# yewsiang/Transferable3D

Measured on AMD Instinct MI355X. Metric: frustums/sec fwd+bwd, higher is better.
Workload: dtype f32

## Files before the change

include/t3d.h:

```cpp
#ifndef T3D_H_
#define T3D_H_

#include <stdint.h>

#ifdef __cplusplus
extern "C" {
#endif

#define T3D_OK 0
#define T3D_ERR_ARG (-1)
#define T3D_ERR_SHAPE (-2)
#define T3D_ERR_LAUNCH (-3)
#define T3D_ERR_ABI (-4)

#define T3D_ABI_VERSION 3
#define T3D_V2_SIZE_pointmlp_fwd_args 200
#define T3D_V2_SIZE_pointmlp_dgrad_args 168
#define T3D_V2_SIZE_pointmlp_wgrad_args 144
#define T3D_V2_SIZE_pointmlp_dgrad_gram_args 168
#define T3D_V2_SIZE_pointmlp_gram_args 96
#define T3D_V2_SIZE_seg_head_args 208
#define T3D_V2_SIZE_boxpc_rep_args 104

#define T3D_TILE_ROWS 128
// ... 694 lines not shown
  float bn_init_decay, bn_decay_rate, bn_decay_step, bn_decay_clip;
  float beta1, beta2;
  int batch_size;
  int step_offset;
} t3d_schedule;
int t3d_schedule_step(float* hyper, const t3d_schedule* s, t3d_stream_t stream);

int t3d_adam_tf_step(float* params, const float* grads, float* m, float* v, int64_t n,
                     const float* hyper, float beta1, float beta2, float eps, float grad_scale,
                     t3d_stream_t stream);

typedef struct { int64_t off; int64_t n; int32_t blk0; int32_t reserved; } t3d_adam_range;
int t3d_reduce_slabs_adam(const float* slab_base, float* grad_base, const t3d_slab_desc* table_dev, int n_tensors, int max_numel,
                          float* params, float* m, float* v, const t3d_adam_range* ranges_dev, int n_ranges, int n_range_blocks,
                          const float* hyper, float beta1, float beta2, float eps, float grad_scale, t3d_stream_t stream);

int t3d_split_x3(const float* src, void* planes, int64_t n, int64_t plane_stride, t3d_stream_t stream);

typedef struct {
  int64_t off;
  int32_t K, N;
  int32_t fwd, dgrad;
  int32_t blk0;
  int32_t reserved;
} t3d_x3_frag_entry;
int t3d_split_x3_frag(const float* params, void* planes_fwd, void* planes_dgrad, int64_t plane_stride, const t3d_x3_frag_entry* table,
                      int n_entries, int n_blocks, t3d_stream_t stream);

int t3d_step_head_takes(const t3d_pointmlp_fwd_args* fwd);
int t3d_step_head(const t3d_pointmlp_fwd_args* fwd, const float* params, void* planes_fwd, void* planes_dgrad, int64_t plane_stride,
                  const t3d_x3_frag_entry* table, int n_entries, int n_blocks, float* hyper, const t3d_schedule* sched,
                  t3d_stream_t stream);

int t3d_momentum_step(float* params, const float* grads, float* accum, int64_t n, const float* hyper, float momentum,
                      float grad_scale, t3d_stream_t stream);

typedef struct {
  t3d_act_src a;
  const float* mask;
  float keep_prob;
  float* out;
  int M, K;
  int rows_per_frustum;
} t3d_act_dropout_args;
int t3d_act_dropout(const t3d_act_dropout_args* args, t3d_stream_t stream);

int t3d_cast_bf16(const float* src, void* dst, int64_t n, t3d_stream_t stream);

int t3d_dropout_mask(float* mask, int64_t n, float keep_prob, uint32_t seed, const float* hyper,
                     t3d_stream_t stream);

enum { T3D_SMALL_BN_BWD_FINALIZE = 1, T3D_SMALL_FC_BWD = 2, T3D_SMALL_FC_DINPUT = 3, T3D_SMALL_DY_COLSUM = 4,
       T3D_SMALL_BN_FWD_FINALIZE = 5, T3D_SMALL_FC_FWD = 6, T3D_SMALL_POOL_BWD_MID = 7 };
typedef struct {
  const float* slab_base;
  float* grad_base;
  const t3d_slab_desc* table_dev;
  int n_tensors, max_numel;
  t3d_pool_sparse_rows_args sparse;
} t3d_pool_bwd_mid_args;
typedef struct {
  int kind;
  int depends;
  union {
    t3d_bn_bwd_finalize_args bn_bwd;
    t3d_fc_bwd_args fc_bwd;
// ... 350 lines not shown
```

transferable3d_amd/abi.py:

```python
import ctypes as C
import os

F = C.POINTER(C.c_float)
I = C.POINTER(C.c_int32)
D = C.POINTER(C.c_double)
L = C.POINTER(C.c_int64)
i32, f32 = C.c_int, C.c_float

TILE_ROWS = 128
F32, BF16 = 0, 1
DTYPE_BY_NAME = {'f32': F32, 'bf16': BF16}
ARITH_AUTO, ARITH_FP32_MFMA, ARITH_BF16X3, ARITH_BF16 = 0, 1, 2, 3
ARITH_BY_NAME = {'auto': ARITH_AUTO, 'fp32_mfma': ARITH_FP32_MFMA, 'bf16x3': ARITH_BF16X3}
ARITH_NAMES = {ARITH_FP32_MFMA: 'fp32_mfma', ARITH_BF16X3: 'bf16x3', ARITH_BF16: 'bf16'}
ABI_VERSION = 3
ERR_ABI = -4
ACT_NONE, ACT_RELU, ACT_LEAKY_RELU, ACT_TANH = 0, 1, 2, 3
ACT_BY_NAME = {None: ACT_NONE, 'relu': ACT_RELU, 'leaky_relu': ACT_LEAKY_RELU, 'tanh': ACT_TANH}


class Sized(C.Structure):

    def __init__(self, *args, **kw):
        super().__init__(C.sizeof(type(self)), *args, **kw)
# ... 7 lines not shown
class DySrc(C.Structure):
    _fields_ = [('dz', F), ('y', F), ('coef', F), ('argidx', I), ('dpool', F), ('dtype', i32)]


class PointMlpFwdArgs(Sized):
    _fields_ = [('struct_size', C.c_uint32), ('a', ActSrc), ('w', F), ('bias', F), ('rowbias', F), ('y', F), ('psum', F), ('psumsq', F),
                ('rowmask', F), ('pmax', F), ('pmin', F), ('pamax', I), ('pamin', I),
                ('M', i32), ('K', i32), ('N', i32), ('rows_per_frustum', i32), ('dtype', i32), ('w_x3', C.c_void_p), ('w_x3_stride', C.c_int64), ('arith', i32)]


class BnFwdFinalizeArgs(C.Structure):
    _fields_ = [('psum', F), ('psumsq', F), ('n_tiles', i32), ('count', i32), ('N', i32), ('gamma', F), ('beta', F),
                ('moving_mean', F), ('moving_var', F), ('decay', F), ('eps', f32), ('is_training', i32),
                ('unbiased_ema', i32), ('scale', F), ('shift', F), ('mean', F), ('invstd', F),
                ('pool_pmax', F), ('pool_pmin', F), ('pool_pamax', I), ('pool_pamin', I), ('pool_B', i32), ('pool_tiles_per_frustum', i32),
                ('pooled', F), ('ld_pooled', i32), ('argidx', I), ('ysel', F)]


class PoolFinalizeArgs(C.Structure):
    _fields_ = [('scale', F), ('shift', F), ('pmax', F), ('pmin', F), ('pamax', I), ('pamin', I),
                ('B', i32), ('N', i32), ('tiles_per_frustum', i32), ('pooled', F), ('ld_pooled', i32),
                ('argidx', I), ('ysel', F)]


class PointMlpDgradArgs(Sized):
    _fields_ = [('struct_size', C.c_uint32), ('dy', DySrc), ('w', F), ('add_in', F), ('prev_y', F), ('prev_scale', F), ('prev_shift', F),
                ('out', F), ('psum_dz', F), ('psum_dzy', F), ('M', i32), ('K', i32), ('N', i32),
                ('rows_per_frustum', i32), ('dtype', i32), ('w_x3', C.c_void_p), ('w_x3_stride', C.c_int64), ('arith', i32)]


class PointMlpWgradArgs(Sized):
    _fields_ = [('struct_size', C.c_uint32), ('a', ActSrc), ('dy', DySrc), ('slabs', F), ('M', i32), ('K', i32), ('N', i32),
                ('rows_per_frustum', i32), ('rows_per_split', i32), ('arith', i32)]


class PoolBwdPrepArgs(C.Structure):
    _fields_ = [('w', F), ('bias', F), ('coef', F), ('K', i32), ('N', i32), ('p_slabs', F), ('rc_slabs', F), ('wc', F)]


class PoolSparseRowsArgs(C.Structure):
    _fields_ = [('argidx', I), ('dpool', F), ('wc', F), ('B', i32), ('N', i32), ('K', i32), ('rows_per_frustum', i32), ('s', F),
                ('row_live', I)]


class PointMlpDgradGramArgs(Sized):
    _fields_ = [('struct_size', C.c_uint32), ('a', ActSrc), ('p', F), ('rowconst', F), ('add_in', F), ('add_live', I), ('prev_y', F), ('prev_scale', F),
                ('prev_shift', F),
                ('out', F), ('psum_dz', F), ('psum_dzy', F), ('M', i32), ('K', i32), ('rows_per_frustum', i32), ('dtype', i32), ('arith', i32)]


class PointMlpGramArgs(Sized):
    _fields_ = [('struct_size', C.c_uint32), ('a', ActSrc), ('slabs', F), ('M', i32), ('K', i32), ('rows_per_frustum', i32), ('rows_per_split', i32), ('arith', i32)]


class ActColsumArgs(C.Structure):
    _fields_ = [('a', ActSrc), ('M', i32), ('K', i32), ('rows_per_frustum', i32), ('part', F)]


class PoolWgradFinishArgs(C.Structure):
    _fields_ = [('a', ActSrc), ('argidx', I), ('dpool', F), ('coef', F), ('w', F), ('bias', F), ('g', F), ('abar', F),
                ('B', i32), ('K', i32), ('N', i32), ('rows_per_frustum', i32), ('dw', F)]


class BoxRefineStepArgs(C.Structure):
    _fields_ = [('out9', F), ('center_in', F), ('dims_in', F), ('theta_in', F), ('center_out', F), ('dims_out', F), ('theta_out', F),
                ('total', F), ('fit_prob', F), ('weigh_by_conf', i32), ('first', i32), ('B', i32)]
# ... 445 lines not shown
    't3d_act_colsum': [C.POINTER(ActColsumArgs), VP],
    't3d_pool_wgrad_finish': [C.POINTER(PoolWgradFinishArgs), VP],
    't3d_batch_assemble': [C.POINTER(BatchAssembleArgs), VP],
    't3d_box_refine_step': [C.POINTER(BoxRefineStepArgs), VP],
    't3d_box_refine_step_bwd': [C.POINTER(BoxRefineStepBwdArgs), VP],
    't3d_boxpc_perturb': [C.POINTER(BoxPcPerturbArgs), VP],
    't3d_sample_equal_classes': [C.POINTER(SampleEqualClassesArgs), VP],
    't3d_box3d_iou': [C.POINTER(Box3dIouArgs), VP],
    't3d_box3d_iou_corners': [C.POINTER(Box3dIouCornersArgs), VP],
    't3d_box_head_iou': [C.POINTER(BoxHeadIouArgs), VP],
    't3d_box2d_feats': [C.POINTER(Box2dFeatsArgs), VP],
    't3d_pool_bwd_stage1': [C.POINTER(PointMlpGramArgs), C.POINTER(ActColsumArgs), C.POINTER(PoolBwdPrepArgs), VP],
    't3d_pool_bwd_mid': [F, F, C.POINTER(SlabDesc), i32, i32, C.POINTER(PoolSparseRowsArgs), VP],
    't3d_pool_bwd_stage2': [C.POINTER(PoolWgradFinishArgs), C.POINTER(PointMlpDgradGramArgs), VP],
    't3d_fc_fwd': [C.POINTER(FcFwdArgs), VP],
    't3d_fc_bwd': [C.POINTER(FcBwdArgs), VP],
    't3d_fc_dinput': [C.POINTER(FcDinputArgs), VP],
    't3d_seg_head': [C.POINTER(SegHeadArgs), VP],
    't3d_seg_finalize': [C.POINTER(SegFinalizeArgs), VP],
    't3d_act_dropout': [C.POINTER(ActDropoutArgs), VP],
    't3d_strong_loss': [C.POINTER(StrongLossArgs), VP],
    't3d_boxpc_rep': [C.POINTER(BoxPcRepArgs), VP],
    't3d_boxpc_rep_b': [C.POINTER(BoxPcRepBArgs), VP],
    't3d_boxpc_rep_bwd': [C.POINTER(BoxPcRepBwdArgs), VP],
    't3d_boxpc_loss': [C.POINTER(BoxPcLossArgs), VP],
    't3d_pointmlp_dgrad_narrow': [C.POINTER(DgradNarrowArgs), VP],
    't3d_semi_final_loss': [C.POINTER(SemiFinalLossArgs), VP],
    't3d_anchor_reg_bwd': [C.POINTER(AnchorRegBwdArgs), VP],
    't3d_reduce_slabs': [F, F, C.POINTER(SlabDesc), i32, i32, VP],
    't3d_schedule_step': [F, C.POINTER(Schedule), VP],
    't3d_reduce_slabs_adam': [F, F, C.POINTER(SlabDesc), i32, i32, F, F, F, C.POINTER(AdamRange), i32, i32, F, f32, f32, f32, f32, VP],
    't3d_step_head_takes': [C.POINTER(PointMlpFwdArgs)],
    't3d_step_head': [C.POINTER(PointMlpFwdArgs), F, VP, VP, C.c_int64, VP, i32, i32, F, C.POINTER(Schedule), VP],
    't3d_adam_tf_step': [F, F, F, F, C.c_int64, F, f32, f32, f32, f32, VP],
    't3d_momentum_step': [F, F, F, C.c_int64, F, f32, f32, VP],
    't3d_split_x3': [F, VP, C.c_int64, C.c_int64, VP],
    't3d_split_x3_frag': [F, VP, VP, C.c_int64, VP, i32, i32, VP],
    't3d_dropout_mask': [F, C.c_int64, f32, C.c_uint32, F, VP],
    't3d_cast_bf16': [F, VP, C.c_int64, VP],
    't3d_frustum_extract': [C.POINTER(FrustumExtractArgs), VP],
    't3d_sunrgbd_eval': [C.POINTER(SunrgbdEvalArgs), VP],
    't3d_sunrgbd_diagnose': [C.POINTER(SunrgbdEvalArgs), C.POINTER(SunrgbdDiagnoseArgs), VP],
    't3d_detect_decode': [C.POINTER(DetectDecodeArgs), VP],
    't3d_detect_nms': [C.POINTER(DetectNmsArgs), VP],
    't3d_render': [C.POINTER(RenderArgs), VP],
    't3d_detect_consistency': [C.POINTER(DetectConsistencyArgs), VP],
    't3d_detect_fuse': [C.POINTER(DetectFuseArgs), VP],
    't3d_detect_ensemble': [C.POINTER(DetectEnsembleArgs), VP],
    't3d_detect_nms_sweep': [C.POINTER(DetectNmsSweepArgs), VP],
    't3d_sunrgbd_eval_sweep': [C.POINTER(SunrgbdEvalArgs), C.POINTER(SunrgbdSweepArgs), VP],
    't3d_semi_sample': [C.POINTER(SemiSampleArgs), VP],
    't3d_label_subset': [C.POINTER(LabelSubsetArgs), VP],
}

LIB_PATH = os.path.join(os.path.dirname(os.path.abspath(__file__)), 'libt3d.so')
ERRORS = {-1: 'T3D_ERR_ARG', -2: 'T3D_ERR_SHAPE', -3: 'T3D_ERR_LAUNCH'}


class T3DError(RuntimeError):
    pass


def source_hash_of(lib):
    buf = C.create_string_buffer(64)
    check(lib.t3d_source_hash(buf, 64), 't3d_source_hash')
    return buf.value.decode()
# ... 46 lines not shown
```

transferable3d_amd/csrc/pointmlp.hip:

```cpp
#include "common.h"
#include "poolbwd_dev.h"
#include "rider_dev.h"

#include <cstdlib>
#include <mutex>
#include <type_traits>
#include <utility>
#include <unordered_map>

namespace {

constexpr int BK = 32;
constexpr int MIN_WAVES_PER_EU = 2;
constexpr int LDR = BK + 4;
constexpr int NT = 256;

__device__ __forceinline__ float4 f4zero() { return make_float4(0.f, 0.f, 0.f, 0.f); }

__device__ __forceinline__ unsigned keep_bits32(const float* __restrict__ rowmask, int base) {
  float4 m[8];
#pragma unroll
  for (int q = 0; q < 8; ++q) m[q] = *reinterpret_cast<const float4*>(rowmask + base + (q >> 2) * 32 + (q & 3) * 8);
  unsigned bits = 0u;
#pragma unroll
// ... 2193 lines not shown
    for (int tn = 0; tn < TN; ++tn) {
      unsigned boff = ((unsigned)(k0 + wm * (BMK / 2) + 4 * h) * (unsigned)N + (unsigned)(n0 + wn * (BN / 2) + tn * 32 + l31)) * 4u;
      asm volatile("" : "+v"(boff));
#pragma unroll
      for (int tm = 0; tm < TM; ++tm)
#pragma unroll
        for (int r = 0; r < 16; ++r)
          *reinterpret_cast<float*>(sbase + (boff + (unsigned)(tm * 32 + (r & 3) + 8 * (r >> 2)) * n4)) = acc[tm][tn][r];
    }
    return;
  }
#pragma unroll
  for (int tn = 0; tn < TN; ++tn) {
    const int col = n0 + wn * (BN / 2) + tn * 32 + l31;
#pragma unroll
    for (int tm = 0; tm < TM; ++tm) {
#pragma unroll
      for (int r = 0; r < 16; ++r) {
        const int k = k0 + wm * (BMK / 2) + tm * 32 + (r & 3) + 8 * (r >> 2) + 4 * h;
        if (k < K) slab[(size_t)k * N + col] = acc[tm][tn][r];
      }
    }
  }
}

template <int BMK, int BN, bool HAS_SUB, bool POOLED, class PR = PathF32, class XT = float>
__global__ __launch_bounds__(NT, MIN_WAVES_PER_EU) void k_pointmlp_wgrad(const t3d_pointmlp_wgrad_args p) {
  extern __shared__ __attribute__((aligned(16))) float smem[];
  typename PR::template Act<HAS_SUB, XT> la{p.a, p.K, p.rows_per_frustum};
  typename PR::template Dy<POOLED> lb{p.dy, p.N, p.rows_per_frustum};
  wgrad_body<BMK, BN, PR>(la, lb, p.slabs, p.K, p.N, p.rows_per_split, smem, blockIdx.x, gridDim.x);
}

template <int N, bool HAS_SUB>
__global__ __launch_bounds__(NT) void k_pointmlp_wgrad_tinyk(const t3d_pointmlp_wgrad_args p) {
  constexpr int CPR = N / 8, RPP = NT / CPR;
  __shared__ float red[RPP][4][N];
  const int tid = threadIdx.x, ch = tid % CPR, r0 = tid / CPR;
  const int split = blockIdx.x, row_begin = split * p.rows_per_split, row_end = row_begin + p.rows_per_split;
  float c0[8], c1[8], c2[8];
#pragma unroll
  for (int e = 0; e < 8; ++e) {
    c0[e] = p.dy.coef[ch * 8 + e];
    c1[e] = p.dy.coef[p.N + ch * 8 + e];
    c2[e] = p.dy.coef[2 * p.N + ch * 8 + e];
  }
  float sc[4] = {1.f, 1.f, 1.f, 1.f}, sh[4] = {0.f, 0.f, 0.f, 0.f};
  if (p.a.scale != nullptr) {
    const float4 a = *reinterpret_cast<const float4*>(p.a.scale), c = *reinterpret_cast<const float4*>(p.a.shift);
    sc[0] = a.x; sc[1] = a.y; sc[2] = a.z; sc[3] = a.w; sh[0] = c.x; sh[1] = c.y; sh[2] = c.z; sh[3] = c.w;
  }
  const float floor_ = p.a.relu ? 0.f : -INFINITY;
  float acc[4][8];
#pragma unroll
  for (int k = 0; k < 4; ++k)
#pragma unroll
    for (int e = 0; e < 8; ++e) acc[k][e] = 0.f;
  constexpr int U = 4;
  for (int r = row_begin + r0; r < row_end; r += RPP * U) {
    float4 dz[U][2], y[U][2], x[U];
#pragma unroll
    for (int u = 0; u < U; ++u) {
      const int rr = min(r + u * RPP, row_end - 1);
      const size_t off = (size_t)rr * p.N + ch * 8;
      dz[u][0] = *reinterpret_cast<const float4*>(p.dy.dz + off);
      dz[u][1] = *reinterpret_cast<const float4*>(p.dy.dz + off + 4);
      y[u][0] = *reinterpret_cast<const float4*>(p.dy.y + off);
      y[u][1] = *reinterpret_cast<const float4*>(p.dy.y + off + 4);
      x[u] = *reinterpret_cast<const float4*>(p.a.x + (size_t)rr * p.a.ldx + p.a.coff);
    }
#pragma unroll
    for (int u = 0; u < U; ++u) {
      const bool live = r + u * RPP < row_end;
      const float xv[4] = {x[u].x, x[u].y, x[u].z, x[u].w};
      float a[4];
      float sub[4] = {0.f, 0.f, 0.f, 0.f};
      if (HAS_SUB) {
        const int b = min(r + u * RPP, row_end - 1) / p.rows_per_frustum;
#pragma unroll
        for (int k = 0; k < 4; ++k) sub[k] = p.a.sub[(size_t)b * p.a.sub_ld + min(k, p.K - 1)];
      }
#pragma unroll
      for (int k = 0; k < 4; ++k) a[k] = (live && k < p.K) ? fmaxf(fmaf(xv[k], sc[k], sh[k]), floor_) - sub[k] : 0.f;
      const float dzv[8] = {dz[u][0].x, dz[u][0].y, dz[u][0].z, dz[u][0].w, dz[u][1].x, dz[u][1].y, dz[u][1].z, dz[u][1].w};
      const float yv[8] = {y[u][0].x, y[u][0].y, y[u][0].z, y[u][0].w, y[u][1].x, y[u][1].y, y[u][1].z, y[u][1].w};
#pragma unroll
      for (int e = 0; e < 8; ++e) {
        const float d = fmaf(c0[e], dzv[e], fmaf(c1[e], yv[e], c2[e]));
#pragma unroll
        for (int k = 0; k < 4; ++k) acc[k][e] = fmaf(a[k], d, acc[k][e]);
      }
    }
  }
#pragma unroll
  for (int k = 0; k < 4; ++k)
#pragma unroll
    for (int e = 0; e < 8; ++e) red[r0][k][ch * 8 + e] = acc[k][e];
  __syncthreads();
  float* slab = p.slabs + (size_t)split * p.K * p.N;
  for (int i = tid; i < p.K * N; i += NT) {
    const int k = i / N, n = i % N;
    float t = 0.f;
#pragma unroll
    for (int g = 0; g < RPP; ++g) t += red[g][k][n];
    slab[(size_t)k * p.N + n] = t;
  }
}

template <int BMK, int BN, class PR = PathF32>
__global__ __launch_bounds__(NT, MIN_WAVES_PER_EU) void k_pointmlp_gram(const t3d_pointmlp_gram_args p) {
  extern __shared__ __attribute__((aligned(16))) float smem[];
  typename PR::template Act<false, typename PR::T> la{p.a, p.K, p.rows_per_frustum};
  wgrad_body<BMK, BN, PR, true>(la, la, p.slabs, p.K, p.K, p.rows_per_split, smem, blockIdx.x, gridDim.x);
}

template <int DBN, int WBMK, int WBN, class PR = PathF32>
__global__ __launch_bounds__(NT, MIN_WAVES_PER_EU) void k_pointmlp_bwd(const t3d_pointmlp_dgrad_args d, const t3d_pointmlp_wgrad_args w,
                                                                const int n_wgrad) {
  extern __shared__ __attribute__((aligned(16))) float smem[];
  typename PR::template Act<false, typename PR::T> la{w.a, w.K, w.rows_per_frustum};
  typename PR::template Dy<false> lb{w.dy, w.N, w.rows_per_frustum};
#ifdef T3D_TRACE
  T3D_TRACE_MARK(0);
  if (threadIdx.x == 0 && t3d_trace_ptr) t3d_trace_ptr[(size_t)blockIdx.x * T3D_TRACE_STRIDE + 1] = (int)blockIdx.x < n_wgrad ? 1 : 2;
#endif
  if ((int)blockIdx.x < n_wgrad) wgrad_body<WBMK, WBN, PR>(la, lb, w.slabs, w.K, w.N, w.rows_per_split, smem, blockIdx.x, n_wgrad);
  else dgrad_body<DBN, false, PR>(d, smem, blockIdx.x - n_wgrad, gridDim.x - n_wgrad);
  T3D_TRACE_MARK(2);
}

template <int DBN, int WBMK, int WBN, class PR = PathF32>
__global__ __launch_bounds__(NT, MIN_WAVES_PER_EU) void k_pointmlp_bwd_r(const t3d_pointmlp_dgrad_args d, const t3d_pointmlp_wgrad_args w,
                                                                  const int n_wgrad, const t3d_rider_set r) {
  extern __shared__ __attribute__((aligned(16))) float smem[];
  if ((int)blockIdx.x < r.n_wg) { run_riders(r, smem); return; }
  const int bid = blockIdx.x - r.n_wg, nblk = gridDim.x - r.n_wg;
  typename PR::template Act<false, float> la{w.a, w.K, w.rows_per_frustum};
  typename PR::template Dy<false> lb{w.dy, w.N, w.rows_per_frustum};
// ... 1630 lines not shown
  if (bwd1_shape(M, K, N, dtype)) {
    static const long target = []() { const char* e = getenv("T3D_BWD1_WGS"); return e ? atol(e) : 256L; }();
    const int tiles = M / 128;
    int per = 1;
    while (tiles / per > target && tiles % (per * 2) == 0) per *= 2;
    if (bwd1_split_ok(M, 128 * per, dtype)) {
      *rows_per_split = 128 * per;
      *one_pass = 1;
      return T3D_OK;
    }
  }
  int tk = 0, tn = 0;
  return t3d_wgrad_plan(M, K, N, rows_per_split, &tk, &tn);
}

static int check_wgrad(const t3d_pointmlp_wgrad_args* a) {
  if (a && a->struct_size != sizeof(*a)) return T3D_ERR_ABI;
  if (!a || !a->slabs || !act_ok(a->a, a->K) || !dy_ok(a->dy)) return T3D_ERR_ARG;
  const int red = a->dy.dtype == T3D_BF16 ? BKH : BK;
  if (a->M <= 0 || a->rows_per_split <= 0 || a->rows_per_split % red || a->M % a->rows_per_split || a->N % 64 ||
      a->rows_per_frustum % red || a->M % a->rows_per_frustum)
    return T3D_ERR_SHAPE;
  if (a->dy.dtype == T3D_F32 && a->a.dtype != T3D_F32) return T3D_ERR_ARG;
  if (a->a.dtype == T3D_BF16 && a->K % 64) return T3D_ERR_SHAPE;
  return T3D_OK;
}
static void wgrad_tile(const t3d_pointmlp_wgrad_args* a, int* tk, int* tn) {
  int rps = 0;
  if (a->M % 128 == 0 && t3d_wgrad_plan(a->M, a->K, a->N, &rps, tk, tn) == T3D_OK && rps == a->rows_per_split) return;
  *tk = a->K > 64 ? 128 : 64;
  *tn = a->N % 128 == 0 ? 128 : 64;
}

extern "C" int t3d_pointmlp_wgrad(const t3d_pointmlp_wgrad_args* a, t3d_stream_t stream) { return t3d_pointmlp_wgrad_r(a, nullptr, stream); }

extern "C" int t3d_pointmlp_wgrad_r(const t3d_pointmlp_wgrad_args* a, const t3d_rider_set* r, t3d_stream_t stream) {
  T3D_ABI_TAKE(pointmlp_wgrad_args, a);
  if (r && !riders_ok(r)) return T3D_ERR_ARG;
  const int rc = check_wgrad(a);
  if (rc != T3D_OK) return rc;
  hipStream_t s = static_cast<hipStream_t>(stream);
  const int splits = a->M / a->rows_per_split;
  int tk = 0, tn = 0;
  wgrad_tile(a, &tk, &tn);
  const int tiles_k = (a->K + tk - 1) / tk, tiles_n = a->N / tn;
  const bool sub = a->a.sub != nullptr, pooled = a->dy.dz == nullptr;
  const bool x3w = a->dy.dtype != T3D_BF16 && a->a.dtype == T3D_F32 && !sub && !pooled && a->K % tk == 0 && a->K % 64 == 0 &&
                   x3_layer_bwd(a->arith, a->K, a->N);
  static const bool use_tiny_w = []() { const char* e = getenv("T3D_WGRAD_TINYK"); return !(e && e[0] == '0'); }();
  const bool tiny_w = use_tiny_w && a->dy.dtype != T3D_BF16 && !pooled && a->K <= 4 && (a->N == 64 || a->N == 128) && a->a.dtype == T3D_F32 &&
                      a->a.ldx % 4 == 0 && a->a.coff % 4 == 0 && a->a.coff + 4 <= a->a.ldx && (a->a.scale == nullptr) == (a->a.shift == nullptr);
  const bool host = r && a->dy.dtype != T3D_BF16 && tk == 64 && tn == 64 && !pooled && !x3w && !tiny_w;
  if (r && !host) { T3D_RIDERS_FIRST(r, stream); r = nullptr; }
  T3D_HOSTED(r, stream);
  const dim3 grid(tiles_k * tiles_n * splits + (r ? r->n_wg : 0));
  if (a->dy.dtype == T3D_BF16) {
    const bool xh = a->a.dtype == T3D_BF16;
#define T3D_WGH(TK, TN_)                                                                                                     \
  do {                                                                                                                       \
    if (sub) launch_lds(k_pointmlp_wgrad<TK, TN_, true, false, PathBF16, float>, grid, lds_wgrad_h(TK, TN_), s, *a);         \
    else if (xh) launch_lds(k_pointmlp_wgrad<TK, TN_, false, false, PathBF16, bf16_t>, grid, lds_wgrad_h(TK, TN_), s, *a);   \
    else launch_lds(k_pointmlp_wgrad<TK, TN_, false, false, PathBF16, float>, grid, lds_wgrad_h(TK, TN_), s, *a);            \
  } while (0)
    if (tk == 128 && tn == 128) T3D_WGH(128, 128);
    else if (tk == 128) T3D_WGH(128, 64);
    else if (tn == 128) T3D_WGH(64, 128);
    else T3D_WGH(64, 64);
#undef T3D_WGH
    T3D_CHECK_LAUNCH();
    return T3D_OK;
  }
#define T3D_WG(TK, TN_)                                                                                   \
  do {                                                                                                    \
    if (sub && pooled) launch_lds(k_pointmlp_wgrad<TK, TN_, true, true>, grid, lds_wgrad(TK, TN_), s, *a);        \
    else if (sub) launch_lds(k_pointmlp_wgrad<TK, TN_, true, false>, grid, lds_wgrad(TK, TN_), s, *a);             \
    else if (pooled) launch_lds(k_pointmlp_wgrad<TK, TN_, false, true>, grid, lds_wgrad(TK, TN_), s, *a);          \
    else launch_lds(k_pointmlp_wgrad<TK, TN_, false, false>, grid, lds_wgrad(TK, TN_), s, *a);                     \
  } while (0)
  if (tiny_w) {
    const dim3 gsp(splits);
    if (a->N == 64) { if (sub) T3D_LAUNCH((k_pointmlp_wgrad_tinyk<64, true>), gsp, dim3(NT), 0, s, *a); else T3D_LAUNCH((k_pointmlp_wgrad_tinyk<64, false>), gsp, dim3(NT), 0, s, *a); }
    else { if (sub) T3D_LAUNCH((k_pointmlp_wgrad_tinyk<128, true>), gsp, dim3(NT), 0, s, *a); else T3D_LAUNCH((k_pointmlp_wgrad_tinyk<128, false>), gsp, dim3(NT), 0, s, *a); }
    T3D_CHECK_LAUNCH();
    return T3D_OK;
// ... 462 lines not shown
```

transferable3d_amd/step.py:

```python
import ctypes as C
import os

import numpy as np
import torch

from . import abi
from .abi import fptr
from .engine import Plan


OPTIMIZER_CALLS = ('t3d_adam_tf_step', 't3d_momentum_step')


class TrainStep:
    def __init__(self, engine, pre, fwd, bwd=None, opt=None, process_group=None, use_hip_graph=None, force_dist=False,
                 one_graph=None, fuse_head_tail=None):
        self.e, self.rt = engine, engine.rt
        if fuse_head_tail is None:
            fuse_head_tail = os.environ.get('T3D_FUSE_HEAD_TAIL', '1') != '0'
        self.fuse_head_tail = bool(fuse_head_tail)
        self.fused = []
        self.pre, self.fwd, self.bwd, self.opt = pre, fwd, bwd, opt
        self.train = bwd is not None
        self.pg = process_group
        self.world = process_group.size() if process_group is not None else 1
        self.dist = self.train and process_group is not None and (self.world > 1 or force_dist)
        self.on_gpu = self.rt.device.type == 'cuda'
        want = use_hip_graph if use_hip_graph is not None else self.on_gpu
        self.want_graph = bool(want) and self.on_gpu
        env = os.environ.get('T3D_DP_ONE_GRAPH', '')
        if one_graph is None:
            if env in ('0', '1', '2'):
                one_graph = env != '0'
            else:
                one_graph = self.dist and self.on_gpu and self._backend() == 'nccl' and self.world == 1
        self.one_graph = bool(one_graph) and self.dist and self.on_gpu
        self.one_graph_form = env if env in ('1', '2') else None
        self.cache = {}
        self.n_runs = 0
        self._capture_stream = None
        self.time_waits = False
        self._wait_events = []
        self._sets = None
        self.schedule_report = None
        self.rider_check_every = int(os.environ.get('T3D_RIDER_CHECK_EVERY', '64'))

    def _backend(self):
        try:
            import torch.distributed as dist
            return str(dist.get_backend(self.pg)).lower()
        except Exception:
            return ''

    def _buckets(self):
        b = list(getattr(self.e, 'buckets', []))
        return b if b else [self.e.default_bucket()]

    def _program(self, generate_masks):
        plans = ([self.pre] if self.pre is not None else []) + [self.fwd] + ([self.bwd, self.opt] if self.train else [])
        calls, lanes, two = [], [], False
        for p in plans:
            for (name, call, arg), lane in zip(p.calls, p.lanes):
                if name == 't3d_dropout_mask' and not generate_masks:
                    continue
                calls.append((name, call, arg))
                lanes.append(lane)
            calls.append((Plan.JOIN, lambda s: 0, None))
            lanes.append(0)
            two = two or p.two_streams
        if self.fuse_head_tail:
            calls, lanes = self._fuse_head_tail(calls, lanes)
        if self.dist and not any(c[0] == Plan.BUCKET for c in calls):
            k = next((i for i, c in enumerate(calls) if c[0] in OPTIMIZER_CALLS), len(calls))
            calls[k:k] = [(Plan.BUCKET, lambda s: 0, 0), (Plan.WAIT, lambda s: 0, 0)]
            lanes[k:k] = [0, 0]
        if not two:
            calls, lanes = self._overlap(calls, lanes)
            two = two or getattr(self, 'two_stream', False)
        prog, cur = [], Plan(self.rt)
        cur.two_streams = two

        def close():
            nonlocal cur
            if len(cur):
                prog.append(('run', cur))
            cur = Plan(self.rt)
            cur.two_streams = two

        for (name, call, arg), lane in zip(calls, lanes):
            if name in (Plan.BUCKET, Plan.WAIT):
                if self.dist:
                    close()
                    prog.append(('allreduce' if name == Plan.BUCKET else 'wait', arg))
                continue
            cur.calls.append((name, call, arg))
            cur.lanes.append(lane)
        close()
        k = len(prog)
        while k > 0 and (prog[k - 1][0] == 'wait' or (prog[k - 1][0] == 'run' and
                                                      all(c[0] in OPTIMIZER_CALLS + (Plan.JOIN,) for c in prog[k - 1][1].calls))):
            k -= 1
        tail = prog[k:]
# ... 33 lines not shown
                    t, n, nblk = vs.frag_table()
                    pf, pd = vs.x3_frag_planes
                    return lib.t3d_step_head(C.byref(a), fptr(vs.params), C.c_void_p(pf.data_ptr()), C.c_void_p(pd.data_ptr()),
                                             vs.x3_frag_stride, C.c_void_p(t.data_ptr()), n, nblk, fptr(hyper), C.byref(sched), s)
                calls[idx[0]] = ('t3d_step_head', head, None)
                drop.update(idx[1:])
                self.fused.append('t3d_step_head')
        idx = adjacent('t3d_reduce_slabs', 't3d_adam_tf_step')
        vs = e.vars
        if idx is not None and self.on_gpu and hasattr(lib, 't3d_reduce_slabs_adam') and not self.dist and e.dt == abi.F32 and \
                names.count('t3d_adam_tf_step') == 1 and idx[1] == real[-1] and getattr(e, 'trained_prefixes', None) is None:
            rd, ad = calls[idx[0]][2], calls[idx[1]][2]
            if (ad['off'], ad['n']) == (0, vs.used) and e.finalized:
                ws = e.ws
                ent = ws.entries[rd['i0']:rd['i1']]
                ranges, nblk = abi.adam_range_table(vs.used, [(go, ne) for _, go, ne, _ in ent])
                host = (abi.AdamRange * max(len(ranges), 1))()
                for i, (off, n, blk0) in enumerate(ranges):
                    host[i] = abi.AdamRange(off, n, blk0, 0)
                table = torch.as_tensor(np.frombuffer(bytes(host), dtype=np.uint8).copy()).to(self.rt.device)
                stride = C.sizeof(abi.SlabDesc)

                def tail(s, rd=rd, ad=ad, table=table, n_ranges=len(ranges), nblk=nblk):
                    return lib.t3d_reduce_slabs_adam(
                        fptr(ws.buf), fptr(vs.grads), C.cast(C.c_void_p(ws.table.data_ptr() + rd['i0'] * stride), C.POINTER(abi.SlabDesc)),
                        rd['i1'] - rd['i0'], rd['max_numel'], fptr(vs.params), fptr(vs.adam_m), fptr(vs.adam_v),
                        C.cast(C.c_void_p(table.data_ptr()), C.POINTER(abi.AdamRange)), n_ranges, nblk, fptr(e.hyper),
                        ad['beta1'], ad['beta2'], ad['eps'], ad['grad_scale'], s)
                calls[idx[0]] = ('t3d_reduce_slabs_adam', tail, None)
                drop.add(idx[1])
                self.fused.append('t3d_reduce_slabs_adam')
        keep = [i for i in range(len(calls)) if i not in drop]
        return [calls[i] for i in keep], [lanes[i] for i in keep]

    def _overlap(self, calls, lanes):
        from . import schedule
        tags = {c[2]: i for i, c in enumerate(calls) if c[0] == Plan.MARK}
        if not all(t in tags for t in ('T_begin', 'S_begin', 'S_end')) or not hasattr(self.rt.lib, 't3d_pointmlp_bwd_r'):
            return calls, lanes
        tb, sb, se = tags['T_begin'], tags['S_begin'], tags['S_end']
        if not tb < sb < se:
            return calls, lanes
        if self._shares_gpu():
            return calls, lanes
        real = lambda cs: [c for c in cs if not c[0].startswith('__')]
        if any(c[0] in (Plan.BUCKET, Plan.WAIT) for c in calls[tb:se]):
            return calls, lanes
        S_calls, T_calls = real(calls[sb:se]), real(calls[tb:sb])
        if self._two_stream_overlap(S_calls + T_calls):
            self.two_stream = True
            first, second = (T_calls, S_calls) if os.environ.get('T3D_TWO_STREAM_FIRST', 'S') == 'T' else (S_calls, T_calls)
            lanes2 = [0] * tb + [1] * len(first) + [0] + [0] * len(second) + [0]
            merged = first + [(Plan.FLUSH, lambda s: 0, None)] + second + [(Plan.JOIN, lambda s: 0, None)]
            calls = calls[:tb] + merged + calls[se + 1:]
            lanes2 += [0] * (len(calls) - len(lanes2))
            self.schedule_report = {'mode': 'two streams', 'S_launches': len(S_calls), 'T_launches': len(T_calls), 'hosted': 0, 'rider_ops': 0,
                                    'pairs': 0, 'solo': len(S_calls) + len(T_calls)}
            return calls, lanes2
        if self._sets is None:
            self._sets = schedule.RiderSets(self.rt)
        merged, self.schedule_report = schedule.overlap_chains(self.rt, S_calls, T_calls, self._sets)
        return calls[:tb] + merged + calls[se + 1:], lanes[:tb] + [0] * len(merged) + lanes[se + 1:]

    def _two_stream_overlap(self, chain_calls):
        mode = os.environ.get('T3D_OVERLAP_STREAMS', '')
        if mode in ('0', '1'):
# ... 340 lines not shown
```

Measured before the change: 28020.

## Batch first-layer tiny-K weight gradients into one launch with recomputed activations

Gathers up to three first-layer weight-gradient calls (K<=4) from the step program and replaces them with one grouped kernel launched just before the slab reduction. Blocks are spread across the problems, largest first. When the matching forward layer is found, the pre-activation output y is recomputed in registers from x, w and bias instead of being read from memory. This removes launch overhead and y reads, but adds scheduling analysis, recompute FLOPs and an assumption that nothing in between touches dz or coef.

```diff
diff --git a/include/t3d.h b/include/t3d.h
--- a/include/t3d.h
+++ b/include/t3d.h
@@ -750,6 +750,16 @@
                   const t3d_x3_frag_entry* table, int n_entries, int n_blocks, float* hyper, const t3d_schedule* sched,
                   t3d_stream_t stream);
 
+typedef struct {
+  uint32_t struct_size;
+  t3d_pointmlp_wgrad_args wgrad;
+  const float* w;
+  const float* bias;
+} t3d_first_layer_wgrad_problem;
+#define T3D_V2_SIZE_first_layer_wgrad_problem 168
+int t3d_first_layer_wgrad(const t3d_first_layer_wgrad_problem* problems, int n_problems, t3d_stream_t stream);
+int t3d_first_layer_wgrad_takes(const t3d_pointmlp_wgrad_args* wgrad, const t3d_pointmlp_fwd_args* fwd);
+
 int t3d_momentum_step(float* params, const float* grads, float* accum, int64_t n, const float* hyper, float momentum,
                       float grad_scale, t3d_stream_t stream);
 
diff --git a/transferable3d_amd/abi.py b/transferable3d_amd/abi.py
--- a/transferable3d_amd/abi.py
+++ b/transferable3d_amd/abi.py
@@ -63,6 +63,10 @@
 class PointMlpWgradArgs(Sized):
     _fields_ = [('struct_size', C.c_uint32), ('a', ActSrc), ('dy', DySrc), ('slabs', F), ('M', i32), ('K', i32), ('N', i32),
                 ('rows_per_frustum', i32), ('rows_per_split', i32), ('arith', i32)]
+
+
+class FirstLayerWgradProblem(Sized):
+    _fields_ = [('struct_size', C.c_uint32), ('wgrad', PointMlpWgradArgs), ('w', F), ('bias', F)]
 
 
 class PoolBwdPrepArgs(C.Structure):
@@ -574,6 +578,8 @@
     't3d_reduce_slabs_adam': [F, F, C.POINTER(SlabDesc), i32, i32, F, F, F, C.POINTER(AdamRange), i32, i32, F, f32, f32, f32, f32, VP],
     't3d_step_head_takes': [C.POINTER(PointMlpFwdArgs)],
     't3d_step_head': [C.POINTER(PointMlpFwdArgs), F, VP, VP, C.c_int64, VP, i32, i32, F, C.POINTER(Schedule), VP],
+    't3d_first_layer_wgrad': [C.POINTER(FirstLayerWgradProblem), i32, VP],
+    't3d_first_layer_wgrad_takes': [C.POINTER(PointMlpWgradArgs), C.POINTER(PointMlpFwdArgs)],
     't3d_adam_tf_step': [F, F, F, F, C.c_int64, F, f32, f32, f32, f32, VP],
     't3d_momentum_step': [F, F, F, C.c_int64, F, f32, f32, VP],
     't3d_split_x3': [F, VP, C.c_int64, C.c_int64, VP],
diff --git a/transferable3d_amd/csrc/pointmlp.hip b/transferable3d_amd/csrc/pointmlp.hip
--- a/transferable3d_amd/csrc/pointmlp.hip
+++ b/transferable3d_amd/csrc/pointmlp.hip
@@ -2249,12 +2249,25 @@
   wgrad_body<BMK, BN, PR>(la, lb, p.slabs, p.K, p.N, p.rows_per_split, smem, blockIdx.x, gridDim.x);
 }
 
-template <int N, bool HAS_SUB>
-__global__ __launch_bounds__(NT) void k_pointmlp_wgrad_tinyk(const t3d_pointmlp_wgrad_args p) {
+template <int N, bool HAS_SUB, bool RECOMP>
+__device__ __forceinline__ void pointmlp_wgrad_tinyk_body(const t3d_pointmlp_wgrad_args& p, const float* __restrict__ wl, const float* __restrict__ bias,
+                                                          float (*red)[4][N], const int split) {
   constexpr int CPR = N / 8, RPP = NT / CPR;
-  __shared__ float red[RPP][4][N];
   const int tid = threadIdx.x, ch = tid % CPR, r0 = tid / CPR;
-  const int split = blockIdx.x, row_begin = split * p.rows_per_split, row_end = row_begin + p.rows_per_split;
+  const int row_begin = split * p.rows_per_split, row_end = row_begin + p.rows_per_split;
+  float w[RECOMP ? 4 : 1][8], add[8];
+  if (RECOMP) {
+#pragma unroll
+    for (int k = 0; k < (RECOMP ? 4 : 1); ++k) {
+      const float4 v0 = *reinterpret_cast<const float4*>(wl + (size_t)min(k, p.K - 1) * p.N + ch * 8);
+      const float4 v1 = *reinterpret_cast<const float4*>(wl + (size_t)min(k, p.K - 1) * p.N + ch * 8 + 4);
+      const float v[8] = {v0.x, v0.y, v0.z, v0.w, v1.x, v1.y, v1.z, v1.w};
+#pragma unroll
+      for (int e = 0; e < 8; ++e) w[k][e] = k < p.K ? v[e] : 0.f;
+    }
+#pragma unroll
+    for (int e = 0; e < 8; ++e) add[e] = bias ? bias[ch * 8 + e] : 0.f;
+  }
   float c0[8], c1[8], c2[8];
 #pragma unroll
   for (int e = 0; e < 8; ++e) {
@@ -2275,15 +2288,17 @@
     for (int e = 0; e < 8; ++e) acc[k][e] = 0.f;
   constexpr int U = 4;
   for (int r = row_begin + r0; r < row_end; r += RPP * U) {
-    float4 dz[U][2], y[U][2], x[U];
+    float4 dz[U][2], y[RECOMP ? 1 : U][2], x[U];
 #pragma unroll
     for (int u = 0; u < U; ++u) {
       const int rr = min(r + u * RPP, row_end - 1);
       const size_t off = (size_t)rr * p.N + ch * 8;
       dz[u][0] = *reinterpret_cast<const float4*>(p.dy.dz + off);
       dz[u][1] = *reinterpret_cast<const float4*>(p.dy.dz + off + 4);
-      y[u][0] = *reinterpret_cast<const float4*>(p.dy.y + off);
-      y[u][1] = *reinterpret_cast<const float4*>(p.dy.y + off + 4);
+      if (!RECOMP) {
+        y[u][0] = *reinterpret_cast<const float4*>(p.dy.y + off);
+        y[u][1] = *reinterpret_cast<const float4*>(p.dy.y + off + 4);
+      }
       x[u] = *reinterpret_cast<const float4*>(p.a.x + (size_t)rr * p.a.ldx + p.a.coff);
     }
 #pragma unroll
@@ -2297,10 +2312,30 @@
 #pragma unroll
         for (int k = 0; k < 4; ++k) sub[k] = p.a.sub[(size_t)b * p.a.sub_ld + min(k, p.K - 1)];
       }
-#pragma unroll
-      for (int k = 0; k < 4; ++k) a[k] = (live && k < p.K) ? fmaxf(fmaf(xv[k], sc[k], sh[k]), floor_) - sub[k] : 0.f;
+      float ay[4];
+#pragma unroll
+      for (int k = 0; k < 4; ++k) {
+        ay[k] = k < p.K ? fmaxf(fmaf(xv[k], sc[k], sh[k]), floor_) - sub[k] : 0.f;
+        a[k] = live ? ay[k] : 0.f;
+      }
       const float dzv[8] = {dz[u][0].x, dz[u][0].y, dz[u][0].z, dz[u][0].w, dz[u][1].x, dz[u][1].y, dz[u][1].z, dz[u][1].w};
-      const float yv[8] = {y[u][0].x, y[u][0].y, y[u][0].z, y[u][0].w, y[u][1].x, y[u][1].y, y[u][1].z, y[u][1].w};
+      float yv[8];
+      if (RECOMP) {
+#pragma clang fp contract(off)
+#pragma unroll
+        for (int e = 0; e < 8; ++e) {
+          float t = ay[0] * w[0][e];
+          t = fmaf(ay[1], w[1][e], t);
+          t = fmaf(ay[2], w[2][e], t);
+          t = fmaf(ay[3], w[3][e], t);
+          yv[e] = t + add[e];
+        }
+      } else {
+        const int yu = RECOMP ? 0 : u;
+        const float yl[8] = {y[yu][0].x, y[yu][0].y, y[yu][0].z, y[yu][0].w, y[yu][1].x, y[yu][1].y, y[yu][1].z, y[yu][1].w};
+#pragma unroll
+        for (int e = 0; e < 8; ++e) yv[e] = yl[e];
+      }
 #pragma unroll
       for (int e = 0; e < 8; ++e) {
         const float d = fmaf(c0[e], dzv[e], fmaf(c1[e], yv[e], c2[e]));
@@ -2321,6 +2356,38 @@
 #pragma unroll
     for (int g = 0; g < RPP; ++g) t += red[g][k][n];
     slab[(size_t)k * p.N + n] = t;
+  }
+}
+
+template <int N, bool HAS_SUB>
+__global__ __launch_bounds__(NT) void k_pointmlp_wgrad_tinyk(const t3d_pointmlp_wgrad_args p) {
+  __shared__ float red[NT / (N / 8)][4][N];
+  pointmlp_wgrad_tinyk_body<N, HAS_SUB, false>(p, nullptr, nullptr, red, blockIdx.x);
+}
+
+struct FirstWgradGroup {
+  t3d_pointmlp_wgrad_args p[3];
+  const float* w[3];
+  const float* bias[3];
+  int end[3];
+};
+__global__ __launch_bounds__(NT) void k_first_layer_wgrad(const FirstWgradGroup g) {
+  __shared__ float red_raw[NT * 4 * 8];
+  const int b = blockIdx.x;
+  const int i = b < g.end[0] ? 0 : (b < g.end[1] ? 1 : 2);
+  const int split = b - (i == 0 ? 0 : g.end[i - 1]);
+  const t3d_pointmlp_wgrad_args& p = g.p[i];
+  const float* w = g.w[i];
+  const float* bias = g.bias[i];
+  const bool sub = p.a.sub != nullptr;
+  auto red64 = reinterpret_cast<float (*)[4][64]>(red_raw);
+  auto red128 = reinterpret_cast<float (*)[4][128]>(red_raw);
+  if (p.N == 64) {
+    if (w) { if (sub) pointmlp_wgrad_tinyk_body<64, true, true>(p, w, bias, red64, split); else pointmlp_wgrad_tinyk_body<64, false, true>(p, w, bias, red64, split); }
+    else { if (sub) pointmlp_wgrad_tinyk_body<64, true, false>(p, w, bias, red64, split); else pointmlp_wgrad_tinyk_body<64, false, false>(p, w, bias, red64, split); }
+  } else {
+    if (w) { if (sub) pointmlp_wgrad_tinyk_body<128, true, true>(p, w, bias, red128, split); else pointmlp_wgrad_tinyk_body<128, false, true>(p, w, bias, red128, split); }
+    else { if (sub) pointmlp_wgrad_tinyk_body<128, true, false>(p, w, bias, red128, split); else pointmlp_wgrad_tinyk_body<128, false, false>(p, w, bias, red128, split); }
   }
 }
 
@@ -4017,7 +4084,73 @@
   *tn = a->N % 128 == 0 ? 128 : 64;
 }
 
+static bool wgrad_takes_tinyk(const t3d_pointmlp_wgrad_args* a) {
+  static const bool use_tiny_w = []() { const char* e = getenv("T3D_WGRAD_TINYK"); return !(e && e[0] == '0'); }();
+  return use_tiny_w && a->dy.dtype != T3D_BF16 && a->dy.dz != nullptr && a->K <= 4 && (a->N == 64 || a->N == 128) && a->a.dtype == T3D_F32 &&
+         a->a.ldx % 4 == 0 && a->a.coff % 4 == 0 && a->a.coff + 4 <= a->a.ldx && (a->a.scale == nullptr) == (a->a.shift == nullptr);
+}
+
 extern "C" int t3d_pointmlp_wgrad(const t3d_pointmlp_wgrad_args* a, t3d_stream_t stream) { return t3d_pointmlp_wgrad_r(a, nullptr, stream); }
+
+static int first_wgrad_check(const t3d_pointmlp_wgrad_args* a) {
+  const int rc = check_wgrad(a);
+  if (rc != T3D_OK) return rc;
+  if (a->dy.dtype != T3D_F32 || a->a.dtype != T3D_F32 || a->dy.dz == nullptr) return T3D_ERR_ARG;
+  if (a->K > 4 || (a->N != 64 && a->N != 128)) return T3D_ERR_SHAPE;
+  return wgrad_takes_tinyk(a) ? T3D_OK : T3D_ERR_ARG;
+}
+
+extern "C" int t3d_first_layer_wgrad_takes(const t3d_pointmlp_wgrad_args* a, const t3d_pointmlp_fwd_args* f) {
+  t3d_pointmlp_wgrad_args al;
+  t3d_pointmlp_fwd_args fl;
+  if (t3d_abi_take(a, al, (uint32_t)T3D_V2_SIZE_pointmlp_wgrad_args) != 0 || first_wgrad_check(a) != T3D_OK) return 0;
+  if (t3d_abi_take(f, fl, (uint32_t)T3D_V2_SIZE_pointmlp_fwd_args) != 0) return 1;
+  if (!f || !f->w || f->dtype != T3D_F32 || f->a.dtype != T3D_F32 || !fwd_takes_tinyk32(f)) return 1;
+  if (f->y != a->dy.y || f->M != a->M || f->K != a->K || f->N != a->N || f->rows_per_frustum != a->rows_per_frustum) return 1;
+  if (f->a.x != a->a.x || f->a.ldx != a->a.ldx || f->a.coff != a->a.coff || f->a.scale != a->a.scale || f->a.shift != a->a.shift ||
+      (f->a.relu != 0) != (a->a.relu != 0) || f->a.sub != a->a.sub || (a->a.sub && f->a.sub_ld != a->a.sub_ld))
+    return 1;
+  if (a->rows_per_frustum % T3D_TILE_ROWS) return 1;
+  return 2;
+}
+
+extern "C" int t3d_first_layer_wgrad(const t3d_first_layer_wgrad_problem* problems, int n_problems, t3d_stream_t stream) {
+  if (!problems || n_problems < 1 || n_problems > 3) return T3D_ERR_ARG;
+  const uint32_t stride = problems->struct_size;
+  t3d_first_layer_wgrad_problem pr[3];
+  int order[3] = {0, 1, 2};
+  for (int i = 0; i < n_problems; ++i) {
+    const t3d_first_layer_wgrad_problem* q =
+        reinterpret_cast<const t3d_first_layer_wgrad_problem*>(reinterpret_cast<const unsigned char*>(problems) + (size_t)i * stride);
+    if (q->struct_size != stride) return T3D_ERR_ABI;
+    T3D_ABI_TAKE(first_layer_wgrad_problem, q);
+    pr[i] = *q;
+    if (pr[i].wgrad.struct_size != sizeof(t3d_pointmlp_wgrad_args)) return T3D_ERR_ABI;
+    const int rc = first_wgrad_check(&pr[i].wgrad);
+    if (rc != T3D_OK) return rc;
+    if ((reinterpret_cast<uintptr_t>(pr[i].w) & 15) || (!pr[i].w && pr[i].bias)) return T3D_ERR_ARG;
+  }
+  auto work = [&](int i) { return (long)pr[i].wgrad.M * pr[i].wgrad.N; };
+  for (int i = 1; i < n_problems; ++i)
+    for (int j = i; j > 0 && work(order[j]) > work(order[j - 1]); --j) { const int t = order[j]; order[j] = order[j - 1]; order[j - 1] = t; }
+  FirstWgradGroup g{};
+  int end = 0;
+  for (int i = 0; i < 3; ++i) {
+    if (i < n_problems) {
+      const t3d_first_layer_wgrad_problem& q = pr[order[i]];
+      g.p[i] = q.wgrad;
+      g.w[i] = q.w;
+      g.bias[i] = q.bias;
+      end += q.wgrad.M / q.wgrad.rows_per_split;
+    } else {
+      g.p[i] = g.p[0];
+    }
+    g.end[i] = end;
+  }
+  T3D_LAUNCH(k_first_layer_wgrad, dim3(end), dim3(NT), 0, static_cast<hipStream_t>(stream), g);
+  T3D_CHECK_LAUNCH();
+  return T3D_OK;
+}
 
 extern "C" int t3d_pointmlp_wgrad_r(const t3d_pointmlp_wgrad_args* a, const t3d_rider_set* r, t3d_stream_t stream) {
   T3D_ABI_TAKE(pointmlp_wgrad_args, a);
@@ -4032,9 +4165,7 @@
   const bool sub = a->a.sub != nullptr, pooled = a->dy.dz == nullptr;
   const bool x3w = a->dy.dtype != T3D_BF16 && a->a.dtype == T3D_F32 && !sub && !pooled && a->K % tk == 0 && a->K % 64 == 0 &&
                    x3_layer_bwd(a->arith, a->K, a->N);
-  static const bool use_tiny_w = []() { const char* e = getenv("T3D_WGRAD_TINYK"); return !(e && e[0] == '0'); }();
-  const bool tiny_w = use_tiny_w && a->dy.dtype != T3D_BF16 && !pooled && a->K <= 4 && (a->N == 64 || a->N == 128) && a->a.dtype == T3D_F32 &&
-                      a->a.ldx % 4 == 0 && a->a.coff % 4 == 0 && a->a.coff + 4 <= a->a.ldx && (a->a.scale == nullptr) == (a->a.shift == nullptr);
+  const bool tiny_w = wgrad_takes_tinyk(a);
   const bool host = r && a->dy.dtype != T3D_BF16 && tk == 64 && tn == 64 && !pooled && !x3w && !tiny_w;
   if (r && !host) { T3D_RIDERS_FIRST(r, stream); r = nullptr; }
   T3D_HOSTED(r, stream);
diff --git a/transferable3d_amd/step.py b/transferable3d_amd/step.py
--- a/transferable3d_amd/step.py
+++ b/transferable3d_amd/step.py
@@ -10,6 +10,30 @@
 
 
 OPTIMIZER_CALLS = ('t3d_adam_tf_step', 't3d_momentum_step')
+
+
+def _pointers(arg):
+    if isinstance(arg, (tuple, list)):
+        for x in arg:
+            yield from _pointers(x)
+    elif isinstance(arg, dict):
+        for x in arg.values():
+            yield from _pointers(x)
+    elif isinstance(arg, C.Array):
+        if issubclass(arg._type_, (C.Structure, C.Union)):
+            for x in arg:
+                yield from _pointers(x)
+    elif isinstance(arg, (C.Structure, C.Union)):
+        for field in arg._fields_:
+            yield from _pointers(getattr(arg, field[0]))
+    elif isinstance(arg, C._Pointer):
+        v = C.cast(arg, C.c_void_p).value
+        if v:
+            yield v
+    elif isinstance(arg, int) and not isinstance(arg, bool):
+        yield arg
+    elif torch.is_tensor(arg):
+        yield arg.data_ptr()
 
 
 class TrainStep:
@@ -20,6 +44,8 @@
             fuse_head_tail = os.environ.get('T3D_FUSE_HEAD_TAIL', '1') != '0'
         self.fuse_head_tail = bool(fuse_head_tail)
         self.fused = []
+        self.fuse_first_wgrad = os.environ.get('T3D_FUSE_FIRST_WGRAD', '1') != '0'
+        self.first_wgrad_fused = False
         self.pre, self.fwd, self.bwd, self.opt = pre, fwd, bwd, opt
         self.train = bwd is not None
         self.pg = process_group
@@ -68,6 +94,7 @@
             calls.append((Plan.JOIN, lambda s: 0, None))
             lanes.append(0)
             two = two or p.two_streams
+        calls, lanes, self.first_wgrad_fused = self._fuse_first_wgrad(calls, lanes) if self.fuse_first_wgrad else (calls, lanes, False)
         if self.fuse_head_tail:
             calls, lanes = self._fuse_head_tail(calls, lanes)
         if self.dist and not any(c[0] == Plan.BUCKET for c in calls):
@@ -167,6 +194,66 @@
                 self.fused.append('t3d_reduce_slabs_adam')
         keep = [i for i in range(len(calls)) if i not in drop]
         return [calls[i] for i in keep], [lanes[i] for i in keep]
+
+    def _fuse_first_wgrad(self, calls, lanes):
+        from . import engine
+        lib, e = self.rt.lib, self.e
+        if not (self.on_gpu and hasattr(lib, 't3d_first_layer_wgrad') and e.dt == abi.F32 and getattr(e, 'finalized', False)) or \
+                engine.DZ_POOL or engine.SIDE_STREAM or engine.FC_SIDE:
+            return calls, lanes, False
+        red = [i for i, c in enumerate(calls) if c[0] == 't3d_reduce_slabs' and isinstance(c[2], dict)]
+        if len(red) != 1:
+            return calls, lanes, False
+        red = red[0]
+        fwd_of, moved = {}, []
+        for i, (name, _, arg) in enumerate(calls[:red]):
+            if name == 't3d_pointmlp_fwd' and isinstance(arg, abi.PointMlpFwdArgs):
+                fwd_of[C.cast(arg.y, C.c_void_p).value] = arg
+            elif name == 't3d_pointmlp_wgrad' and isinstance(arg, abi.PointMlpWgradArgs):
+                f = fwd_of.get(C.cast(arg.dy.y, C.c_void_p).value)
+                takes = lib.t3d_first_layer_wgrad_takes(C.byref(arg), C.byref(f) if f is not None else None)
+                if takes in (1, 2):
+                    moved.append((i, arg, f if takes == 2 else None))
+        moved = moved[-3:]
+        if not moved:
+            return calls, lanes, False
+        first = moved[0][0]
+        if any(c[0] in (Plan.BUCKET, Plan.WAIT) or c[0] in OPTIMIZER_CALLS for c in calls[first:red]):
+            return calls, lanes, False
+        taken = {i for i, _, _ in moved}
+        inside = lambda p, spans: any(lo <= p < lo + n for lo, n in spans)
+        for i in range(first + 1, red):
+            name, _, arg = calls[i]
+            if i in taken:
+                continue
+            behind = [a for j, a, _ in moved if j < i]
+            dz = [(C.cast(a.dy.dz, C.c_void_p).value, 4 * a.M * a.N) for a in behind]
+            coef = [(C.cast(a.dy.coef, C.c_void_p).value, 4 * 3 * a.N) for a in behind]
+            assert not any(inside(p, dz) for p in _pointers(arg)), \
+                '%s between a first layer\'s weight gradient and the slab reduction points into its dz' % name
+            for x in (arg if isinstance(arg, (tuple, list)) else (arg,)):
+                if isinstance(x, abi.BnBwdFinalizeArgs):
+                    assert not inside(C.cast(x.coef, C.c_void_p).value or 0, coef), \
+                        '%s between a first layer\'s weight gradient and the slab reduction writes its coef' % name
+        group = (abi.FirstLayerWgradProblem * len(moved))()
+        for k, (_, a, f) in enumerate(moved):
+            C.memmove(C.byref(group[k].wgrad), C.byref(a), C.sizeof(a))
+            group[k].struct_size = C.sizeof(abi.FirstLayerWgradProblem)
+            if f is not None:
+                group[k].w, group[k].bias = f.w, f.bias
+        n = len(moved)
+
+        def launch(s, group=group, n=n):
+            return lib.t3d_first_layer_wgrad(group, n, s)
+        keep = [i for i in range(len(calls)) if i not in taken]
+        out, out_lanes = [], []
+        for i in keep:
+            if i == red:
+                out.append(('t3d_first_layer_wgrad', launch, None))
+                out_lanes.append(0)
+            out.append(calls[i])
+            out_lanes.append(lanes[i])
+        return out, out_lanes, True
 
     def _overlap(self, calls, lanes):
         from . import schedule
```

Result: no change. 28170 (median of 6 runs) (+0.5%).
